# nyasyamorina/font-renderer

Measured on AMD Instinct MI355X. Metric: Mpixel/s AA glyph coverage, higher is better.
Workload: dtype f32

## Files before the change

### bindings/fr_raster.zig

```
const std = @import("std");

const Font = @import("../font/Font.zig");
const Glyph = @import("../font/Glyph.zig");
const Image = @import("Image.zig");
const Point = @import("geometry.zig").Point;

pub const fr_ctx = opaque {};
pub const fr_glyphset = opaque {};
pub const fr_plan = opaque {};
pub const fr_font = opaque {};

pub const Status = enum(c_int) { ok = 0, invalid = -1, hip = -2, nomem = -3, unsupported = -4 };
pub const Mode = enum(i32) { winding_i16 = 0, gray_debug = 1, mask_nonzero = 2, coverage_u8 = 3, sdf_u8 = 4 };
pub const SamplePhase = enum(i32) { corner = 0, center = 1 };
pub const FR_FONT_ALLOW_HINTED: u32 = 1;
pub const FR_FILL_CONSISTENT: u32 = 1;
pub const FR_TEXT_BGRA: u32 = 4;
pub const FR_TEXT_SRGB: u32 = 8;
pub const FR_TEXT_LOAD: u32 = 32;

pub const RasterParams = extern struct {
    mode: i32,
    samples_per_axis: i32,
    sample_phase: i32,
// ... 78 lines not shown
pub extern "c" fn fr_font_close(font: ?*fr_font) void;
pub extern "c" fn fr_font_info(font: *const fr_font, units_per_em: ?*u16, num_glyphs: ?*u16, y0_baseline: ?*c_int) c_int;
pub extern "c" fn fr_font_char_to_glyph(font: *const fr_font, codepoint: u32, glyph_index: *u16) c_int;
pub extern "c" fn fr_font_glyph_advance(font: *const fr_font, glyph_index: u16, advance_width: *i16) c_int;
pub extern "c" fn fr_text_layout(font: *const fr_font, codepoints: [*]const u32, n: u32, font_size: u16, glyph_index_out: [*]u16, pen_x64_out: [*]i32, end_pen_x64: ?*i32) c_int;
pub extern "c" fn fr_font_glyph_measure(font: *fr_font, glyph_index: u16, n_contours: *u32, n_points: *u32, box: *[4]i16) c_int;
pub extern "c" fn fr_font_glyph_fill(font: *fr_font, glyph_index: u16, points_xy: [*]i16, contour_start: [*]u32) c_int;
pub extern "c" fn fr_qoi_bound(width: u32, height: u32) usize;
pub extern "c" fn fr_qoi_encode_rgb(rgb: [*]const u8, width: u32, height: u32, out: [*]u8, cap: usize, n_out: *usize) c_int;
pub extern "c" fn fr_qoi_encode_gray(gray: [*]const u8, width: u32, height: u32, stride: usize, out: [*]u8, cap: usize, n_out: *usize) c_int;
pub extern "c" fn fr_qoi_encode_rgba(rgba: [*]const u8, width: u32, height: u32, stride_px: usize, out: [*]u8, cap: usize, n_out: *usize) c_int;
pub extern "c" fn fr_srgb_decode(in: [*]const u8, n: usize, out: [*]u16) c_int;
pub extern "c" fn fr_srgb_encode(in: [*]const u16, n: usize, out: [*]u8) c_int;
pub extern "c" fn fr_selftest_division(d_lo: u32, d_hi: u32, mismatches: *u64, bad_divisor: ?*u32, bad_x_bits: ?*u32) c_int;
pub extern "c" fn fr_selftest_sqrt(mismatches: *u64, bad_x_bits: ?*u32) c_int;

pub const Error = error{ RasterFailed, OutOfMemory };

var g_ctx: ?*fr_ctx = null;

fn context() Error!*fr_ctx {
    if (g_ctx == null) {
        if (fr_ctx_create(0, null, &g_ctx) != 0) return error.RasterFailed;
    }
    return g_ctx.?;
}

pub fn deinit() void {
    if (g_ctx) |c| fr_ctx_destroy(c);
    g_ctx = null;
// ... 131 lines not shown
```

### font-renderer_amd/_lib.py

```python
from __future__ import annotations

import ctypes as C
import os

FR_WINDING_I16, FR_GRAY_DEBUG, FR_MASK_NONZERO, FR_COVERAGE_U8, FR_SDF_U8 = 0, 1, 2, 3, 4
FR_SAMPLE_CORNER, FR_SAMPLE_CENTER = 0, 1
FR_FILL_CONSISTENT = 1
FR_TEXT_SRGB, FR_TEXT_BGRA = 8, 4
FR_TEXT_LOAD = 32

_HERE = os.path.dirname(os.path.abspath(__file__))


def lib_path() -> str:
    return os.environ.get("FR_RASTER_LIB") or os.path.join(_HERE, "libfr_raster.so")


class FrError(RuntimeError):
    def __init__(self, code: int, msg: str):
        super().__init__(f"fr_raster error {code}: {msg}")
        self.code = code


class Job(C.Structure):
# ... 73 lines not shown
    ("fr_font_open", C.c_int, [_P, C.c_size_t, C.c_uint32, C.POINTER(_P)]),
    ("fr_font_close", None, [_P]),
    ("fr_font_info", C.c_int, [_P, C.POINTER(C.c_uint16), C.POINTER(C.c_uint16), C.POINTER(C.c_int)]),
    ("fr_font_char_to_glyph", C.c_int, [_P, C.c_uint32, C.POINTER(C.c_uint16)]),
    ("fr_font_glyph_advance", C.c_int, [_P, C.c_uint16, C.POINTER(C.c_int16)]),
    ("fr_text_layout", C.c_int, [_P, _P, C.c_uint32, C.c_uint16, _P, _P, C.POINTER(C.c_int32)]),
    ("fr_font_glyph_measure", C.c_int, [_P, C.c_uint16, C.POINTER(C.c_uint32), C.POINTER(C.c_uint32), _P]),
    ("fr_font_glyph_fill", C.c_int, [_P, C.c_uint16, _P, _P]),
    ("fr_qoi_bound", C.c_size_t, [C.c_uint32, C.c_uint32]),
    ("fr_qoi_encode_rgb", C.c_int, [_P, C.c_uint32, C.c_uint32, _P, C.c_size_t, C.POINTER(C.c_size_t)]),
    ("fr_qoi_encode_gray", C.c_int, [_P, C.c_uint32, C.c_uint32, C.c_size_t, _P, C.c_size_t, C.POINTER(C.c_size_t)]),
    ("fr_qoi_encode_rgba", C.c_int, [_P, C.c_uint32, C.c_uint32, C.c_size_t, _P, C.c_size_t, C.POINTER(C.c_size_t)]),
    ("fr_srgb_decode", C.c_int, [_P, C.c_size_t, _P]),
    ("fr_srgb_encode", C.c_int, [_P, C.c_size_t, _P]),
    ("fr_selftest_sqrt", C.c_int, [C.POINTER(C.c_uint64), C.POINTER(C.c_uint32)]),
    ("fr_selftest_division", C.c_int, [C.c_uint32, C.c_uint32, C.POINTER(C.c_uint64), C.POINTER(C.c_uint32), C.POINTER(C.c_uint32)]),
]

_lib = None


def _preload_hip_runtime() -> None:
    if os.environ.get("FR_HIP_RUNTIME", "") == "system":
        return
    import importlib.util
    import sys
    if "torch" in sys.modules:
        return
    try:
        spec = importlib.util.find_spec("torch")
# ... 35 lines not shown
```

### font-renderer_amd/csrc/fr_c4.hpp

```cpp
#pragma once
#include "fr_records.hpp"
#include "fr_wave.hpp"

namespace fr {

#ifndef FR_C4_WAVES
#define FR_C4_WAVES 4
#endif
#ifndef FR_C4_OCC
#define FR_C4_OCC 4
#endif
#ifndef FR_C4_PCAP
#define FR_C4_PCAP 448
#endif
#ifndef FR_C4_OCC_SMALL
#define FR_C4_OCC_SMALL 6
#endif
#ifndef FR_DYN_BANDS
#define FR_DYN_BANDS 1
#endif
#ifndef FR_W1_OCC_SMALL
#define FR_W1_OCC_SMALL 6
#endif
enum { C4_WAVES = FR_C4_WAVES, C4_PCAP = FR_C4_PCAP };
constexpr uint32_t c4_lstride(int cap) { return (uint32_t)cap + 4u; }
constexpr int c4_occ(int cap, int wlog, int rpl) { return rpl >= 16 ? 2 : (rpl >= 8 ? 3 : ((cap <= 16 && rpl == 2) ? FR_C4_OCC_SMALL : FR_C4_OCC)); }
constexpr int w1_occ(int rpl, int wlog) { return rpl >= 16 ? 2 : ((rpl == 2) ? FR_W1_OCC_SMALL : FR_C4_OCC); }
template <uint32_t LSTRIDE>
__device__ __forceinline__ uint4 c4_ld16(const uint16_t *p)
{
    if ((LSTRIDE * 2) % 16 == 0) return *reinterpret_cast<const uint4 *>(p);
    const uint2 a = reinterpret_cast<const uint2 *>(p)[0], b = reinterpret_cast<const uint2 *>(p)[1];
    return make_uint4(a.x, a.y, b.x, b.y);
}
// ... 37 lines not shown
__device__ __forceinline__ Rec40 c4_make_rec40(const Rec &r, uint32_t ra, uint32_t re)
{
    Rec40 m;
    const bool lin = (int32_t)r.flags < 0;
    m.a = lin ? r.c1 : r.a;
    m.b = r.b; m.c1 = lin ? 0.0f : r.c1; m.c2 = r.c2;
    m.ax = r.ax; m.bx = r.bx; m.p0x = r.p0x; m.rden = r.rden;
    m.sgn = r.sqsign ? -1.0f : 1.0f;
    const uint32_t cb = (lin || FILL) ? (r.flags & 2u) : 2u, zb = (lin || FILL) ? cb : 0u;
    m.fr = ra | (re << 12) | (cb << 24) | (zb << 26) | (lin ? 0x80000000u : 0u);
    return m;
}

template <uint32_t RCAP, int N, uint32_t NCOL, int FILL>
__device__ __forceinline__ uint32_t c4_setup_small(const RenderArgs &A, const Job &job, uint32_t seg0, uint32_t nseg, uint32_t x0s,
                                                   int phase, float *s_cxp, Rec40 *s_rec, uint32_t *s_wcnt, uint32_t *s_tmp, const float *cyt = nullptr)
{
    const uint32_t tid = threadIdx.x, lane = tid & 63u, wave = tid >> 6;
    const uint32_t Hs = job.h * (uint32_t)N;
    RowGeom geo;
    geo.max_y = job.max_y; geo.scale = job.scale; geo.rows = Hs; geo.n = N; geo.phase = phase; geo.cyt = cyt;
    const bool have = lane < 2u * nseg;
    Rec r;
    RowGuess g;
    Piece pc;
    g.empty = true; g.ra = 1u; g.re = 0u;
    uint32_t cls = 3u;
    if (have) {
        record_prep<FILL>(A.seg_pts + 6u * (size_t)(seg0 + (lane >> 1)), lane & 1u, geo, r, g, &pc);
        if (!g.empty) {
            const uint32_t row = (wave == 0u) ? g.ra - 1u : (wave == 1u) ? g.ra : (wave == 2u) ? g.re - 1u : g.re;
            if (row < Hs && (wave != 2u || g.re > g.ra)) cls = (uint32_t)row_class<FILL>(r, pc, geo.cy(row));
        }
    }
    s_tmp[tid] = cls;
    const int32_t min_xs = job.min_x + (int32_t)x0s;
    for (uint32_t j = tid; j < NCOL; j += 256u)
        s_cxp[1u + j] = ((float)(min_xs + (int32_t)(j / (uint32_t)N)) + sub_off((int)(j % (uint32_t)N), N, phase)) / job.scale;
    if (tid == 2) s_cxp[0] = -__builtin_inff();
    if (tid == 3) s_cxp[1u + NCOL] = __builtin_inff();
    __syncthreads();
    if (wave == 0u) {
        Rec40 mine;
        mine.fr = 0u;
        bool live = false;
        if (have) {
            uint32_t ra = g.ra, re = g.re;
            if (!g.empty) {
                const uint32_t c0 = s_tmp[lane], c1 = s_tmp[64u + lane], c2 = s_tmp[128u + lane], c3 = s_tmp[192u + lane];
                const bool ok = (c0 >= 2u) && (c1 <= 1u || c1 == 3u) && re >= ra && (c2 >= 1u) && (c3 == 0u || c3 == 3u);
                if (!ok) record_settle<FILL>(r, geo, ra, re, &pc);
            }
            live = ra < re;
// ... 2 lines not shown
        const bool linr = live && (int32_t)mine.fr < 0;
        const unsigned long long lm = __ballot(live && !linr), ll = __ballot(linr), below = (1ull << lane) - 1ull;
        const uint32_t n_quad = (uint32_t)__popcll(lm);
        uint32_t pos = RCAP;
        if ((lm >> lane) & 1ull) pos = (uint32_t)__popcll(lm & below);
        if ((ll >> lane) & 1ull) pos = n_quad + (uint32_t)__popcll(ll & below);
        if (pos < RCAP) s_rec[pos] = mine;
        if (lane == 0u) s_wcnt[0] = min(n_quad + (uint32_t)__popcll(ll), RCAP);
    }
    __syncthreads();
    return s_wcnt[0];
}

template <uint32_t RCAP, int N, uint32_t NCOL, int FILL>
__device__ __forceinline__ uint32_t c4_setup_mid(const RenderArgs &A, const Job &job, uint32_t seg0, uint32_t nseg, uint32_t x0s,
                                                 int phase, float *s_cxp, Rec40 *s_rec, uint32_t *s_wcnt, uint32_t *s_tmp, const float *cyt = nullptr)
{
    const uint32_t tid = threadIdx.x, lane = tid & 63u, wave = tid >> 6;
    const uint32_t c = tid & 127u, h = tid >> 7;
    const uint32_t Hs = job.h * (uint32_t)N;
    RowGeom geo;
    geo.max_y = job.max_y; geo.scale = job.scale; geo.rows = Hs; geo.n = N; geo.phase = phase; geo.cyt = cyt;
    const bool have = c < 2u * nseg;
    Rec r;
    RowGuess g;
    Piece pc;
    g.empty = true; g.ra = 1u; g.re = 0u;
    uint32_t cls0 = 3u, cls1 = 3u;
    if (have) {
        record_prep<FILL>(A.seg_pts + 6u * (size_t)(seg0 + (c >> 1)), c & 1u, geo, r, g, &pc);
        if (!g.empty) {
            const uint32_t end = h ? g.re : g.ra;
            if (end - 1u < Hs && (h == 0u || g.re > g.ra)) cls0 = (uint32_t)row_class<FILL>(r, pc, geo.cy(end - 1u));
            if (end < Hs) cls1 = (uint32_t)row_class<FILL>(r, pc, geo.cy(end));
        }
    }
    s_tmp[tid] = cls0 | (cls1 << 8);
    const int32_t min_xs = job.min_x + (int32_t)x0s;
    for (uint32_t j = tid; j < NCOL; j += 256u)
        s_cxp[1u + j] = ((float)(min_xs + (int32_t)(j / (uint32_t)N)) + sub_off((int)(j % (uint32_t)N), N, phase)) / job.scale;
    if (tid == 2) s_cxp[0] = -__builtin_inff();
    if (tid == 3) s_cxp[1u + NCOL] = __builtin_inff();
    __syncthreads();
    Rec40 mine;
    mine.fr = 0u;
    bool live = false;
    if (h == 0u && have) {
        uint32_t ra = g.ra, re = g.re;
        if (!g.empty) {
            const uint32_t up = s_tmp[c], dn = s_tmp[128u + c];
            const uint32_t c0 = up & 0xffu, c1 = up >> 8, c2 = dn & 0xffu, c3 = dn >> 8;
            const bool ok = (c0 >= 2u) && (c1 <= 1u || c1 == 3u) && re >= ra && (c2 >= 1u) && (c3 == 0u || c3 == 3u);
            if (!ok) record_settle<FILL>(r, geo, ra, re, &pc);
        }
        live = ra < re;
// ... 1 lines not shown
    }
    const bool linr = live && (int32_t)mine.fr < 0;
    const unsigned long long lm = __ballot(live && !linr), ll = __ballot(linr), below = (1ull << lane) - 1ull;
    if (lane == 0u && wave < 2u) { s_wcnt[wave] = (uint32_t)__popcll(lm); s_wcnt[2u + wave] = (uint32_t)__popcll(ll); }
    __syncthreads();
    const uint32_t q0 = s_wcnt[0], q1 = s_wcnt[1], l0 = s_wcnt[2], l1 = s_wcnt[3];
    const uint32_t n_quad = q0 + q1;
    uint32_t pos = RCAP;
    if ((lm >> lane) & 1ull) pos = (wave ? q0 : 0u) + (uint32_t)__popcll(lm & below);
    if ((ll >> lane) & 1ull) pos = n_quad + (wave ? l0 : 0u) + (uint32_t)__popcll(ll & below);
    if (wave < 2u && pos < RCAP) s_rec[pos] = mine;
    __syncthreads();
    return min(n_quad + l0 + l1, RCAP);
}

template <uint32_t NW, uint32_t RCAP, int N, uint32_t NCOL, int FILL = 0>
__device__ __forceinline__ uint32_t c4_setup(const RenderArgs &A, const Job &job, uint32_t seg0, uint32_t nseg, uint32_t x0s,
                                             int phase, float *s_cxp, Rec40 *s_rec, uint32_t *s_wcnt, uint32_t *s_tmp, const float *cyt = nullptr)
{
    if (NW == 4u && 2u * nseg <= 64u)
        return c4_setup_small<RCAP, N, NCOL, FILL>(A, job, seg0, nseg, x0s, phase, s_cxp, s_rec, s_wcnt, s_tmp, cyt);
    if (NW == 4u && 2u * nseg <= 128u)
        return c4_setup_mid<RCAP, N, NCOL, FILL>(A, job, seg0, nseg, x0s, phase, s_cxp, s_rec, s_wcnt, s_tmp, cyt);
    const uint32_t tid = threadIdx.x, lane = tid & 63u, wave = tid >> 6;
    const uint32_t Hs = job.h * (uint32_t)N;
    constexpr uint32_t CPT = (RCAP >= 1024u ? 1536u : (RCAP >= 512u ? 768u : 512u)) / (64u * NW);
    s_wcnt = s_tmp;
    Rec40 mine[CPT];
    unsigned long long lm[CPT], ll[CPT];
#pragma unroll
    for (uint32_t it = 0; it < CPT; ++it) {
        const uint32_t c = tid + it * 64u * NW;
        bool live = false;
        lm[it] = 0ull; ll[it] = 0ull;
        mine[it].fr = 0u;
        if (it > 0 && it * 64u * NW >= 2u * nseg) continue;
        if (c < 2u * nseg) {
            Rec r;
            RowGeom geo;
            geo.max_y = job.max_y; geo.scale = job.scale; geo.rows = Hs; geo.n = N; geo.phase = phase; geo.cyt = cyt;
            build_record_rows<FILL>(A.seg_pts + 6u * (size_t)(seg0 + (c >> 1)), c & 1u, geo, r);
            const uint32_t ra = __builtin_bit_cast(uint32_t, r.lo), re = __builtin_bit_cast(uint32_t, r.hi);
            live = ra < re;
            mine[it] = c4_make_rec40<FILL>(r, ra, re);
        }
        const bool linr = live && (int32_t)mine[it].fr < 0;
        lm[it] = __ballot(live && !linr);
        ll[it] = __ballot(linr);
        if (lane == 0) { s_wcnt[it * NW + wave] = (uint32_t)__popcll(lm[it]); s_wcnt[CPT * NW + it * NW + wave] = (uint32_t)__popcll(ll[it]); }
    }
    const int32_t min_xs = job.min_x + (int32_t)x0s;
    for (uint32_t j = tid; j < NCOL; j += 64u * NW)
        s_cxp[1u + j] = ((float)(min_xs + (int32_t)(j / (uint32_t)N)) + sub_off((int)(j % (uint32_t)N), N, phase)) / job.scale;
    if (tid == 2) s_cxp[0] = -__builtin_inff();
    if (tid == 3) s_cxp[1u + NCOL] = __builtin_inff();
    __syncthreads();
    uint32_t rec_cnt = 0;
    {
        uint32_t base_q[CPT], base_l[CPT], n_quad = 0;
#pragma unroll
        for (uint32_t it = 0; it < CPT; ++it) base_q[it] = base_l[it] = 0;
#pragma unroll
        for (uint32_t q = 0; q < CPT * NW; ++q) {
            if (q >= NW && q / NW * 64u * NW >= 2u * nseg) continue;
            const uint32_t cq = s_wcnt[q], cl = s_wcnt[CPT * NW + q];
#pragma unroll
            for (uint32_t it = 0; it < CPT; ++it) {
                base_q[it] += (q < it * NW + wave) ? cq : 0u;
// ... 21 lines not shown
```

### font-renderer_amd/csrc/fr_cov4_kernel.inc

```
    using L = C4Lds<WLOG, RPL, NS, CAP>;
    constexpr uint32_t LSTRIDE = L::LSTRIDE;
    static_assert(NS == 4 || NS == 2, "samples per axis");
    constexpr uint32_t RCAP = L::RCAP;
    constexpr uint32_t NW = C4_WAVES;
    constexpr uint32_t SW = 16u << WLOG;
    constexpr uint32_t NCOL = SW * (uint32_t)NS;
    constexpr uint32_t NWIN = 1u << WLOG;
    constexpr uint32_t PRB = L::PRB;
    constexpr int LN = (NS == 4) ? 2 : 1;
    constexpr bool SPLIT = RPL >= 8 && CAP == 32;
    extern __shared__ __align__(16) unsigned char smem[];

    const uint32_t tid = threadIdx.x, lane = tid & 63u;
    const uint32_t wave = (uint32_t)__builtin_amdgcn_readfirstlane((int)(tid >> 6));
    uint32_t bid = blockIdx.x, strip = 0, bgrp = 0;
    if (A.strips != 1u) { strip = bid % A.strips; bid /= A.strips; }
    if (A.band_groups != 1u) { bgrp = bid % A.band_groups; bid /= A.band_groups; }
    const uint32_t jidx = bid;
    C4_ABL_LAUNCH_ONLY();
    const Job job = A.jobs[jidx];
    const uint32_t x0s = strip * SW;
    const uint32_t band_first = bgrp * A.bands_per_wg;
    if (band_first * PRB >= job.h || x0s >= job.w) return;
    const uint32_t band_end = min(band_first + A.bands_per_wg, (job.h + PRB - 1u) / PRB);
    const uint32_t wlim = min(SW, job.w - x0s);
    const int phase = A.phase_center;
    const uint32_t seg0 = A.job_seg[2u * (size_t)jidx], nseg = A.job_seg[2u * (size_t)jidx + 1u];
    C4_ABL_JOB_ONLY();
    C4_ABL_SEGLOAD_ONLY();
    float *s_cxp = reinterpret_cast<float *>(smem);
    Rec40 *s_rec = reinterpret_cast<Rec40 *>(smem + L::CX);
    unsigned char *wregion = smem + L::OFF_WAVES + (size_t)wave * L::WAVE;
    uint32_t *s_wcnt = reinterpret_cast<uint32_t *>(smem + L::OFF_WCNT);

    uint32_t *const s_next_band = s_wcnt + 15;
    if (tid == 0u) *s_next_band = band_first + NW;
    const uint32_t rec_cnt = c4_setup<NW, RCAP, NS, NCOL, FILL>(A, job, seg0, nseg, x0s, phase, s_cxp, s_rec, s_wcnt, reinterpret_cast<uint32_t *>(smem + L::OFF_WAVES));
    const int32_t min_xs = job.min_x + (int32_t)x0s;
    const float jscale = job.scale * (float)NS;
    const float joff = (float)min_xs * (float)NS + (phase ? 0.5f : 0.0f) - 1.0f;
    const float ncolf = (float)NCOL;
    const bool few = RPL == 2 || rec_cnt <= 128u;
    const uint32_t per = few ? 2u : (uint32_t)RPL;
    uint32_t rra[RPL], rre[RPL];
#pragma unroll
    for (int i = 0; i < RPL; ++i) {
        const uint32_t k = per * lane + (uint32_t)i;
        const bool have = k < rec_cnt && (!few || i < 2);
        const uint32_t f = s_rec[have ? k : 0u].fr;
        rra[i] = have ? (f & 0xfffu) : 1u;
        rre[i] = have ? ((f >> 12) & 0xfffu) : 0u;
    }
// ... 4 lines not shown
    uint32_t *s_cnt = reinterpret_cast<uint32_t *>(wregion + L::OFF_CNT);
    int16_t *s_roff = reinterpret_cast<int16_t *>(wregion + L::OFF_ROFF);
    unsigned char *s_E = wregion;

    C4_ABL_SETUP_ONLY();
#if FR_DYN_BANDS
    for (uint32_t band = band_first + wave; band < band_end;
         band = (uint32_t)__builtin_amdgcn_readfirstlane((int)(lane == 0u ? atomicAdd(s_next_band, 1u) : 0u))) {
#else
    for (uint32_t band0 = band_first; band0 < band_end; band0 += NW) {
        const uint32_t band = band0 + wave;
        if (band >= band_end) break;
#endif
        const uint32_t y0 = band * PRB;
        const uint32_t row_b0 = band * 64u;
        const float cy = ((float)(job.max_y - (int32_t)(y0 + (lane >> LN))) - sub_off((int)(lane & (uint32_t)(NS - 1)), NS, phase)) / job.scale;
        uint16_t *mylist = s_lists + lane * LSTRIDE;
        auto init_lists = [&]() {
            const uint4 ones = make_uint4(0xfffdfffdu, 0xfffdfffdu, 0xfffdfffdu, 0xfffdfffdu);
#pragma unroll
            for (uint32_t q = 0; q < CAP / 8u; ++q) c4_st16<LSTRIDE>(mylist + 8u * q, ones);
            s_cnt[lane] = 0u;
        };
        init_lists();
        s_cy[lane] = cy;

        uint32_t c[RPL], off0 = 0u, tot;
        {
            uint32_t r0[RPL], csum = 0;
            {
                const uint32_t lo = row_b0, hi = row_b0 + 64u;
// ... 442 lines not shown
```

### font-renderer_amd/csrc/fr_device.hpp

```cpp
#pragma once
#include <hip/hip_runtime.h>
#include <stdint.h>

#pragma clang fp contract(off)

namespace fr {

struct __attribute__((aligned(16))) Rec {
    float lo, hi, a, b, c1, c2, ax, bx, p0x;
    uint32_t flags;
    float rden;
    uint32_t sqsign;
};

__device__ __forceinline__ float div_by_int(float x, float d, float rd)
{
    const float q = x * rd;
    const float r = __builtin_fmaf(-q, d, x);
    return __builtin_fmaf(r, rd, q);
}
__device__ __forceinline__ float sqrt_rn(float x)
{
    const float s = __builtin_amdgcn_sqrtf(x);
    const float sm = __builtin_bit_cast(float, __builtin_bit_cast(int, s) - 1);
    const float sp = __builtin_bit_cast(float, __builtin_bit_cast(int, s) + 1);
    const float rm = __builtin_fmaf(-sm, s, x);
    const float rp = __builtin_fmaf(-sp, s, x);
    float r = (rm <= 0.0f) ? sm : s;
    r = (rp > 0.0f) ? sp : r;
    return r;
}
enum : uint32_t {
    REC_LINEAR = 0x80000000u,
    REC_NEG_ROOT = 2u,
// ... 123 lines not shown
```

### font-renderer_amd/csrc/fr_records.hpp

```cpp
#pragma once
#include "fr_device.hpp"

namespace fr {

__device__ __forceinline__ int classify(const Rec &r, float cy)
{
    if (r.flags & REC_LINEAR) {
        float t = rec_t_lin(r, cy);
        bool up = r.c1 > 0.0f;
        if (t < 0.0f) return up ? 0 : 2;
        if (t >= 1.0f) return up ? 2 : 0;
        return 1;
    }
    float delta = cy * r.a + r.c1 - r.c2;
    if (delta < 0.0f) return (r.a > 0.0f) ? 0 : 2;
    float t = rec_t_quad(r, cy);
    bool neg = (r.flags & REC_NEG_ROOT) != 0;
    if (t < 0.0f) return neg ? 2 : 0;
    if (t >= 1.0f) return neg ? 0 : 2;
    return 1;
}

__device__ __noinline__ uint32_t first_at_least(float ra, float rb, float rc1, float rc2, uint32_t rflags, int T, uint32_t L, uint32_t H)
{
// ... 77 lines not shown
        r.rden = 1.0f / a;
        r.flags = root ? REC_NEG_ROOT : 0u;
    }
    float lo, hi;
    if (!accept_bracket(r, p0y, p2y, lo, hi)) return false;
    r.lo = lo; r.hi = hi;
    return true;
}

struct RowGeom {
    int32_t max_y;
    float scale;
    uint32_t rows;
    int n, phase;
    const float *cyt = nullptr;
    __device__ __forceinline__ float cy(uint32_t r) const
    {
        if (cyt) return cyt[r];
        return ((float)(max_y - (int32_t)(r / (uint32_t)n)) - sub_off((int)(r % (uint32_t)n), n, phase)) / scale;
    }
    __device__ __forceinline__ float row_of(float c) const
    {
        return ((float)max_y - c * scale) * (float)n - (phase ? 0.5f : 0.0f);
    }
};

__device__ __forceinline__ int classify_row(const Rec &r, float cy)
{
    const bool lin = (r.flags & REC_LINEAR) != 0;
    const float delta = cy * r.a + r.c1 - r.c2;
    const float sq = sqrt_rn(delta);
    const float num = lin ? (cy - r.b) : ((r.flags & REC_NEG_ROOT) ? (r.b - sq) : (r.b + sq));
    const float t = div_by_int(num, lin ? r.c1 : r.a, r.rden);
    const bool falls = lin ? !(r.c1 > 0.0f) : ((r.flags & REC_NEG_ROOT) != 0);
// ... 164 lines not shown
```

### font-renderer_amd/csrc/fr_selftest.hip

```cpp
#include "../../include/fr_raster.h"
#include "fr_device.hpp"

namespace fr {

__global__ __launch_bounds__(256) void selftest_div_kernel(uint32_t d_lo, uint32_t n_d,
                                                           unsigned long long *mismatches,
                                                           uint32_t *first_bad)
{
    const uint32_t d_idx = blockIdx.x / 32u, part = blockIdx.x % 32u;
    if (d_idx >= n_d) return;
    const float d = (float)(d_lo + d_idx);
    const float rd = 1.0f / d, rdn = 1.0f / (-d);
    uint32_t bad = 0, bad_x = 0;
    for (uint32_t m = part * 256u + threadIdx.x; m < (1u << 23); m += 32u * 256u) {
        const float x = __uint_as_float(0x3f800000u | m);
        const float xs = __uint_as_float(0x2f800000u | m);
        const float xl = __uint_as_float(0x4f800000u | m);
        const bool ok = (__float_as_uint(div_by_int(x, d, rd)) == __float_as_uint(x / d)) &&
                        (__float_as_uint(div_by_int(x, -d, rdn)) == __float_as_uint(x / -d)) &&
                        (__float_as_uint(div_by_int(-xs, d, rd)) == __float_as_uint(-xs / d)) &&
                        (__float_as_uint(div_by_int(xl, d, rd)) == __float_as_uint(xl / d));
        if (!ok) { ++bad; bad_x = 0x3f800000u | m; }
    }
    if (bad) {
// ... 3 lines not shown
    }
}

__global__ __launch_bounds__(256) void selftest_sqrt_kernel(uint32_t e_lo, unsigned long long *mismatches, uint32_t *first_bad)
{
    const uint32_t e = e_lo + blockIdx.x / 32u, part = blockIdx.x % 32u;
    uint32_t bad = 0, bad_x = 0;
    for (uint32_t m = part * 256u + threadIdx.x; m < (1u << 23); m += 32u * 256u) {
        const uint32_t bits = (e << 23) | m;
        const float x = __uint_as_float(bits);
        if (__float_as_uint(sqrt_rn(x)) != __float_as_uint(__builtin_sqrtf(x))) { ++bad; bad_x = bits; }
    }
    if (bad) {
        atomicAdd(mismatches, (unsigned long long)bad);
        first_bad[0] = bad_x;
    }
}

}

extern "C" int fr_selftest_sqrt(uint64_t *mismatches, uint32_t *bad_x_bits)
{
    if (!mismatches) return FR_E_INVALID;
    unsigned long long *d_m = nullptr;
    uint32_t *d_b = nullptr;
    if (hipMalloc(&d_m, 8) != hipSuccess || hipMalloc(&d_b, 8) != hipSuccess) return FR_E_HIP;
    (void)hipMemset(d_m, 0, 8);
    (void)hipMemset(d_b, 0, 8);
    const uint32_t e_lo = 97u, e_hi = 192u;
    hipLaunchKernelGGL(fr::selftest_sqrt_kernel, dim3((e_hi - e_lo + 1u) * 32u), dim3(256), 0, 0, e_lo, d_m, d_b);
// ... 23 lines not shown
        const uint32_t n = n_d - off < 4096u ? n_d - off : 4096u;
        hipLaunchKernelGGL(fr::selftest_div_kernel, dim3(n * 32u), dim3(256), 0, 0, d_lo + off, n, d_m, d_b);
    }
    unsigned long long m = 0;
    uint32_t b[2] = {0, 0};
    hipError_t e = hipMemcpy(&m, d_m, 8, hipMemcpyDeviceToHost);
    if (e == hipSuccess) e = hipMemcpy(b, d_b, 8, hipMemcpyDeviceToHost);
    (void)hipFree(d_m);
    (void)hipFree(d_b);
    if (e != hipSuccess) return FR_E_HIP;
    *mismatches = m;
    if (bad_divisor) *bad_divisor = b[0];
    if (bad_x_bits) *bad_x_bits = b[1];
    return FR_OK;
}
```

### font-renderer_amd/csrc/fr_win1_kernel.inc

```
    using L = W1Lds<WLOG, RPL>;
    constexpr uint32_t NW = C4_WAVES;
    constexpr uint32_t RCAP = L::RCAP;
    constexpr uint32_t NCOL = L::NCOL;
    constexpr uint32_t NWIN = 1u << WLOG;
    constexpr uint32_t PCAP = L::PCAP;
    constexpr uint32_t ESZ = (MODE == MODE1_WINDING_I16) ? 2u : 1u;
    extern __shared__ __align__(16) unsigned char smem[];

    const uint32_t tid = threadIdx.x, lane = tid & 63u;
    const uint32_t wave = (WLOG == 4 && RPL == 2) ? (tid >> 6) : (uint32_t)__builtin_amdgcn_readfirstlane((int)(tid >> 6));
    uint32_t bid = blockIdx.x, strip = 0, bgrp = 0;
    if (A.strips != 1u) { strip = bid % A.strips; bid /= A.strips; }
    if (A.band_groups != 1u) { bgrp = bid % A.band_groups; bid /= A.band_groups; }
    const uint32_t jidx = bid;
    const Job job = A.jobs[jidx];
    const uint32_t x0s = strip * NCOL;
    const uint32_t band_first = bgrp * A.bands_per_wg;
    if (band_first * W1_ROWS >= job.h || x0s >= job.w) return;
    const uint32_t band_end = min(band_first + A.bands_per_wg, (job.h + W1_ROWS - 1u) / W1_ROWS);
    const uint32_t wlim = min(NCOL, job.w - x0s);
    const int phase = A.phase_center;
    const uint32_t seg0 = A.job_seg[2u * (size_t)jidx], nseg = A.job_seg[2u * (size_t)jidx + 1u];

    float *s_cxp = reinterpret_cast<float *>(smem);
    Rec40 *s_rec = reinterpret_cast<Rec40 *>(smem + L::CX);
    unsigned char *wregion = smem + L::OFF_WAVES + (size_t)wave * L::WAVE;
    uint32_t *s_wcnt = reinterpret_cast<uint32_t *>(smem + L::OFF_WCNT);

    const float soff = phase ? 0.5f : 0.0f;
    const float *cyt = nullptr;
    if (job.h <= 256u) {
        float *t = reinterpret_cast<float *>(smem + L::OFF_CYT);
        if (tid < job.h) t[tid] = ((float)(job.max_y - (int32_t)tid) - soff) / job.scale;
        __syncthreads();
        cyt = t;
    }
    const uint32_t rec_cnt_v = c4_setup<NW, RCAP, 1, NCOL, FILL>(A, job, seg0, nseg, x0s, phase, s_cxp, s_rec, s_wcnt, reinterpret_cast<uint32_t *>(smem + L::OFF_WAVES), cyt);
    const uint32_t rec_cnt = (WLOG == 4 && RPL == 2) ? rec_cnt_v : (uint32_t)__builtin_amdgcn_readfirstlane((int)rec_cnt_v);
    const int32_t min_xs = job.min_x + (int32_t)x0s;
    const float jscale = job.scale;
    const float joff = (float)min_xs + soff - 1.0f;
    const float ncolf = (float)NCOL;
    const bool few = RPL == 2 || rec_cnt <= 128u;
    const uint32_t per = few ? 2u : (uint32_t)RPL;
    uint32_t rra[RPL], rre[RPL];
#pragma unroll
    for (int i = 0; i < RPL; ++i) {
        const uint32_t k = per * lane + (uint32_t)i;
        const bool have = k < rec_cnt && (!few || i < 2);
        const uint32_t f = s_rec[have ? k : 0u].fr;
        rra[i] = have ? (f & 0xfffu) : 1u;
        rre[i] = have ? ((f >> 12) & 0xfffu) : 0u;
    }

    unsigned char *s_E = wregion;
    uint16_t *s_pairs = reinterpret_cast<uint16_t *>(wregion + L::OFF_PAIRS);
    float *s_cy = reinterpret_cast<float *>(wregion + L::OFF_CY);
    uint32_t *s_cnt = reinterpret_cast<uint32_t *>(wregion + L::OFF_CNT);
    int16_t *s_roff = reinterpret_cast<int16_t *>(wregion + L::OFF_ROFF);
    const uint32_t wx = lane & (NWIN - 1u);

    for (uint32_t band0 = band_first; band0 < band_end; band0 += NW) {
        const uint32_t band = band0 + wave;
        if (band >= band_end) break;
        const uint32_t y0 = band * W1_ROWS;
        const float cy = cyt ? cyt[y0 + (lane & 15u)] : ((float)(job.max_y - (int32_t)(y0 + (lane & 15u))) - soff) / job.scale;
        {
            uint4 *z = reinterpret_cast<uint4 *>(s_E);
            const uint4 bias = make_uint4(0x20202020u, 0x20202020u, 0x20202020u, 0x20202020u);
            constexpr uint32_t NZ = L::E / 16u;
#pragma unroll
            for (uint32_t q = 0; q < (NZ + 63u) / 64u; ++q)
                if (NZ % 64u == 0u || lane + 64u * q < NZ) z[lane + 64u * q] = bias;
        }
        if (lane < 16u) { s_cy[lane] = cy; s_cnt[lane] = 0u; }

        uint32_t rr0 = 0;
        while (rr0 < W1_ROWS) {
            uint32_t span = W1_ROWS - rr0;
            uint32_t c[RPL], r0[RPL], csum, incl, tot;
            for (;;) {
// ... 330 lines not shown
```

### include/fr_raster.h

```cpp
#ifndef FR_RASTER_H
#define FR_RASTER_H

#include <stddef.h>
#include <stdint.h>

#ifdef __cplusplus
extern "C" {
#endif

#define FR_ABI_VERSION 1

typedef enum fr_status {
    FR_OK = 0,
    FR_E_INVALID = -1,
    FR_E_HIP = -2,
    FR_E_NOMEM = -3,
    FR_E_UNSUPPORTED = -4
} fr_status;

typedef enum fr_mode {
    FR_WINDING_I16 = 0,
    FR_GRAY_DEBUG = 1,
    FR_MASK_NONZERO = 2,
    FR_COVERAGE_U8 = 3,
// ... 150 lines not shown

int fr_text_layout(const fr_font *font, const uint32_t *codepoints, uint32_t n, uint16_t font_size,
                   uint16_t *glyph_index_out, int32_t *pen_x64_out, int32_t *end_pen_x64);

size_t fr_qoi_bound(uint32_t width, uint32_t height);
int fr_qoi_encode_rgb(const uint8_t *rgb, uint32_t width, uint32_t height, uint8_t *out, size_t cap, size_t *n_out);
int fr_qoi_encode_gray(const uint8_t *gray, uint32_t width, uint32_t height, size_t stride, uint8_t *out, size_t cap, size_t *n_out);
int fr_qoi_encode_rgba(const uint8_t *rgba, uint32_t width, uint32_t height, size_t stride_px, uint8_t *out, size_t cap, size_t *n_out);

int fr_srgb_decode(const uint8_t *in, size_t n, uint16_t *out);
int fr_srgb_encode(const uint16_t *in, size_t n, uint8_t *out);

int fr_selftest_division(uint32_t d_lo, uint32_t d_hi, uint64_t *mismatches,
                         uint32_t *bad_divisor, uint32_t *bad_x_bits);
int fr_selftest_sqrt(uint64_t *mismatches, uint32_t *bad_x_bits);

#ifdef __cplusplus
}
#endif
#endif
```

Baseline: 2.489 million.

## Replace per-row scale divisions with reciprocal refinement and add dense setup path

Replaces the IEEE float divisions by job.scale in row and column coordinate setup with a wave-uniform reciprocal plus two FMA correction steps meant to match division exactly, and adds a selftest that checks this bitwise against true division. It also adds a dense setup path in the cov4 kernel for glyphs with up to 256 segments. That path compacts live records per wave with ballots, then classifies endpoint rows in parallel before settling. The aim is to cut division latency and the serialized setup work per job, at the cost of more code and reliance on the exactness of the refinement.

```diff
diff --git a/bindings/fr_raster.zig b/bindings/fr_raster.zig
--- a/bindings/fr_raster.zig
+++ b/bindings/fr_raster.zig
@@ -116,6 +116,7 @@
 pub extern "c" fn fr_srgb_encode(in: [*]const u16, n: usize, out: [*]u8) c_int;
 pub extern "c" fn fr_selftest_division(d_lo: u32, d_hi: u32, mismatches: *u64, bad_divisor: ?*u32, bad_x_bits: ?*u32) c_int;
 pub extern "c" fn fr_selftest_sqrt(mismatches: *u64, bad_x_bits: ?*u32) c_int;
+pub extern "c" fn fr_selftest_scale_division(mismatches: *u64, bad_scale_bits: ?*u32, bad_x_bits: ?*u32) c_int;
 
 pub const Error = error{ RasterFailed, OutOfMemory };
 
diff --git a/font-renderer_amd/_lib.py b/font-renderer_amd/_lib.py
--- a/font-renderer_amd/_lib.py
+++ b/font-renderer_amd/_lib.py
@@ -111,6 +111,7 @@
     ("fr_srgb_decode", C.c_int, [_P, C.c_size_t, _P]),
     ("fr_srgb_encode", C.c_int, [_P, C.c_size_t, _P]),
     ("fr_selftest_sqrt", C.c_int, [C.POINTER(C.c_uint64), C.POINTER(C.c_uint32)]),
+    ("fr_selftest_scale_division", C.c_int, [C.POINTER(C.c_uint64), C.POINTER(C.c_uint32), C.POINTER(C.c_uint32)]),
     ("fr_selftest_division", C.c_int, [C.c_uint32, C.c_uint32, C.POINTER(C.c_uint64), C.POINTER(C.c_uint32), C.POINTER(C.c_uint32)]),
 ]
 
diff --git a/font-renderer_amd/csrc/fr_c4.hpp b/font-renderer_amd/csrc/fr_c4.hpp
--- a/font-renderer_amd/csrc/fr_c4.hpp
+++ b/font-renderer_amd/csrc/fr_c4.hpp
@@ -18,6 +18,9 @@
 #endif
 #ifndef FR_DYN_BANDS
 #define FR_DYN_BANDS 1
+#endif
+#ifndef FR_C4_DENSE
+#define FR_C4_DENSE 1
 #endif
 #ifndef FR_W1_OCC_SMALL
 #define FR_W1_OCC_SMALL 6
@@ -85,12 +88,12 @@
 
 template <uint32_t RCAP, int N, uint32_t NCOL, int FILL>
 __device__ __forceinline__ uint32_t c4_setup_small(const RenderArgs &A, const Job &job, uint32_t seg0, uint32_t nseg, uint32_t x0s,
-                                                   int phase, float *s_cxp, Rec40 *s_rec, uint32_t *s_wcnt, uint32_t *s_tmp, const float *cyt = nullptr)
+                                                   int phase, float ysc, float *s_cxp, Rec40 *s_rec, uint32_t *s_wcnt, uint32_t *s_tmp, const float *cyt = nullptr)
 {
     const uint32_t tid = threadIdx.x, lane = tid & 63u, wave = tid >> 6;
     const uint32_t Hs = job.h * (uint32_t)N;
     RowGeom geo;
-    geo.max_y = job.max_y; geo.scale = job.scale; geo.rows = Hs; geo.n = N; geo.phase = phase; geo.cyt = cyt;
+    geo.max_y = job.max_y; geo.scale = job.scale; geo.rows = Hs; geo.n = N; geo.phase = phase; geo.cyt = cyt; geo.by_rcp = true; geo.yscale = ysc;
     const bool have = lane < 2u * nseg;
     Rec r;
     RowGuess g;
@@ -107,7 +110,7 @@
     s_tmp[tid] = cls;
     const int32_t min_xs = job.min_x + (int32_t)x0s;
     for (uint32_t j = tid; j < NCOL; j += 256u)
-        s_cxp[1u + j] = ((float)(min_xs + (int32_t)(j / (uint32_t)N)) + sub_off((int)(j % (uint32_t)N), N, phase)) / job.scale;
+        s_cxp[1u + j] = div_by_scale((float)(min_xs + (int32_t)(j / (uint32_t)N)) + sub_off((int)(j % (uint32_t)N), N, phase), job.scale, ysc);
     if (tid == 2) s_cxp[0] = -__builtin_inff();
     if (tid == 3) s_cxp[1u + NCOL] = __builtin_inff();
     __syncthreads();
@@ -140,13 +143,13 @@
 
 template <uint32_t RCAP, int N, uint32_t NCOL, int FILL>
 __device__ __forceinline__ uint32_t c4_setup_mid(const RenderArgs &A, const Job &job, uint32_t seg0, uint32_t nseg, uint32_t x0s,
-                                                 int phase, float *s_cxp, Rec40 *s_rec, uint32_t *s_wcnt, uint32_t *s_tmp, const float *cyt = nullptr)
+                                                 int phase, float ysc, float *s_cxp, Rec40 *s_rec, uint32_t *s_wcnt, uint32_t *s_tmp, const float *cyt = nullptr)
 {
     const uint32_t tid = threadIdx.x, lane = tid & 63u, wave = tid >> 6;
     const uint32_t c = tid & 127u, h = tid >> 7;
     const uint32_t Hs = job.h * (uint32_t)N;
     RowGeom geo;
-    geo.max_y = job.max_y; geo.scale = job.scale; geo.rows = Hs; geo.n = N; geo.phase = phase; geo.cyt = cyt;
+    geo.max_y = job.max_y; geo.scale = job.scale; geo.rows = Hs; geo.n = N; geo.phase = phase; geo.cyt = cyt; geo.by_rcp = true; geo.yscale = ysc;
     const bool have = c < 2u * nseg;
     Rec r;
     RowGuess g;
@@ -164,7 +167,7 @@
     s_tmp[tid] = cls0 | (cls1 << 8);
     const int32_t min_xs = job.min_x + (int32_t)x0s;
     for (uint32_t j = tid; j < NCOL; j += 256u)
-        s_cxp[1u + j] = ((float)(min_xs + (int32_t)(j / (uint32_t)N)) + sub_off((int)(j % (uint32_t)N), N, phase)) / job.scale;
+        s_cxp[1u + j] = div_by_scale((float)(min_xs + (int32_t)(j / (uint32_t)N)) + sub_off((int)(j % (uint32_t)N), N, phase), job.scale, ysc);
     if (tid == 2) s_cxp[0] = -__builtin_inff();
     if (tid == 3) s_cxp[1u + NCOL] = __builtin_inff();
     __syncthreads();
@@ -196,14 +199,119 @@
     return min(n_quad + l0 + l1, RCAP);
 }
 
-template <uint32_t NW, uint32_t RCAP, int N, uint32_t NCOL, int FILL = 0>
+template <uint32_t RCAP, int N, uint32_t NCOL, uint32_t WAVE>
+__device__ __forceinline__ uint32_t c4_setup_dense(const RenderArgs &A, const Job &job, uint32_t seg0, uint32_t nseg, uint32_t x0s,
+                                                   int phase, float ysc, float *s_cxp, Rec40 *s_rec, uint32_t *s_wcnt, unsigned char *s_waves)
+{
+    constexpr uint32_t LIST = 128u * (uint32_t)sizeof(Rec40);
+    static_assert(RCAP == 256u && WAVE >= LIST + RCAP * 4u, "no room for the dense root lists");
+    const uint32_t tid = threadIdx.x, lane = tid & 63u, wave = tid >> 6;
+    const uint32_t Hs = job.h * (uint32_t)N;
+    const unsigned long long below = (1ull << lane) - 1ull;
+    RowGeom geo;
+    geo.max_y = job.max_y; geo.scale = job.scale; geo.rows = Hs; geo.n = N; geo.phase = phase; geo.by_rcp = true; geo.yscale = ysc;
+    uint32_t *s_cls = reinterpret_cast<uint32_t *>(s_waves + LIST);
+    auto rec_of = [](const Rec40 &m) {
+        Rec r;
+        const bool lin = (int32_t)m.fr < 0;
+        r.a = lin ? 0.0f : m.a; r.b = m.b; r.c1 = lin ? m.a : m.c1; r.c2 = m.c2; r.rden = m.rden;
+        r.flags = lin ? (uint32_t)REC_LINEAR : (m.sgn < 0.0f ? (uint32_t)REC_NEG_ROOT : 0u);
+        return r;
+    };
+    {
+        Rec40 e0, e1;
+        bool live0 = false, live1 = false;
+        if (tid < nseg) {
+            const int16_t *p = A.seg_pts + 6u * (size_t)(seg0 + tid);
+            Rec r;
+            RowGuess g;
+            record_prep<0>(p, 0u, geo, r, g);
+            live0 = !g.empty;
+            e0 = c4_make_rec40<0>(r, g.ra, g.re);
+            record_prep<0>(p, 1u, geo, r, g);
+            live1 = !g.empty;
+            e1 = c4_make_rec40<0>(r, g.ra, g.re);
+        }
+        const unsigned long long m0 = __ballot(live0), m1 = __ballot(live1);
+        Rec40 *mylist = reinterpret_cast<Rec40 *>(s_waves + (size_t)wave * WAVE);
+        const uint32_t pos = (uint32_t)__popcll(m0 & below) + (uint32_t)__popcll(m1 & below);
+        if (live0) mylist[pos] = e0;
+        if (live1) mylist[pos + (live0 ? 1u : 0u)] = e1;
+        if (lane == 0u) s_wcnt[wave] = (uint32_t)__popcll(m0) + (uint32_t)__popcll(m1);
+    }
+    const int32_t min_xs = job.min_x + (int32_t)x0s;
+    for (uint32_t j = tid; j < NCOL; j += 256u)
+        s_cxp[1u + j] = div_by_scale((float)(min_xs + (int32_t)(j / (uint32_t)N)) + sub_off((int)(j % (uint32_t)N), N, phase), job.scale, ysc);
+    if (tid == 2) s_cxp[0] = -__builtin_inff();
+    if (tid == 3) s_cxp[1u + NCOL] = __builtin_inff();
+    __syncthreads();
+    const uint32_t cum0 = s_wcnt[0], cum1 = cum0 + s_wcnt[1], cum2 = cum1 + s_wcnt[2];
+    const uint32_t nl = min(cum2 + s_wcnt[3], RCAP);
+    auto entry = [&](uint32_t j) {
+        const uint32_t w = (j >= cum0 ? 1u : 0u) + (j >= cum1 ? 1u : 0u) + (j >= cum2 ? 1u : 0u);
+        const uint32_t first = w == 0u ? 0u : (w == 1u ? cum0 : (w == 2u ? cum1 : cum2));
+        return reinterpret_cast<const Rec40 *>(s_waves + (size_t)w * WAVE) + (j - first);
+    };
+    for (uint32_t i = tid; i < 2u * nl; i += 256u) {
+        const Rec40 *ep = entry(i >> 1);
+        Rec40 m;
+        m.a = ep->a; m.b = ep->b; m.c1 = ep->c1; m.c2 = ep->c2; m.rden = ep->rden; m.sgn = ep->sgn; m.fr = ep->fr;
+        const Rec r = rec_of(m);
+        const Piece pc{};
+        const uint32_t ra = m.fr & 0xfffu, re = (m.fr >> 12) & 0xfffu;
+        const uint32_t end = (i & 1u) ? re : ra;
+        uint32_t cls0 = 3u, cls1 = 3u;
+        if (end - 1u < Hs && ((i & 1u) == 0u || re > ra)) cls0 = (uint32_t)row_class<0>(r, pc, geo.cy(end - 1u));
+        if (end < Hs) cls1 = (uint32_t)row_class<0>(r, pc, geo.cy(end));
+        reinterpret_cast<uint16_t *>(s_cls)[i] = (uint16_t)(cls0 | (cls1 << 8));
+    }
+    __syncthreads();
+    Rec40 mine = {};
+    bool live = false;
+    if (tid < nl) {
+        const Rec40 *ep = entry(tid);
+        mine.a = ep->a; mine.b = ep->b; mine.c1 = ep->c1; mine.c2 = ep->c2; mine.ax = ep->ax; mine.bx = ep->bx; mine.p0x = ep->p0x;
+        mine.rden = ep->rden; mine.sgn = ep->sgn; mine.fr = ep->fr;
+        uint32_t ra = mine.fr & 0xfffu, re = (mine.fr >> 12) & 0xfffu;
+        const uint32_t c4 = s_cls[tid];
+        const uint32_t c0 = c4 & 0xffu, c1 = (c4 >> 8) & 0xffu, c2 = (c4 >> 16) & 0xffu, c3 = c4 >> 24;
+        const bool ok = (c0 >= 2u) && (c1 <= 1u || c1 == 3u) && re >= ra && (c2 >= 1u) && (c3 == 0u || c3 == 3u);
+        if (!ok) record_settle<0>(rec_of(mine), geo, ra, re);
+        live = ra < re;
+        mine.fr = (mine.fr & 0xff000000u) | ra | (re << 12);
+    }
+    const bool linr = live && (int32_t)mine.fr < 0;
+    const unsigned long long lm = __ballot(live && !linr), ll = __ballot(linr);
+    if (lane == 0u) { s_wcnt[4u + wave] = (uint32_t)__popcll(lm); s_wcnt[8u + wave] = (uint32_t)__popcll(ll); }
+    __syncthreads();
+    uint32_t base_q = 0u, base_l = 0u, n_quad = 0u, n_lin = 0u;
+#pragma unroll
+    for (uint32_t w = 0; w < 4u; ++w) {
+        const uint32_t cq = s_wcnt[4u + w], cl = s_wcnt[8u + w];
+        base_q += (w < wave) ? cq : 0u;
+        base_l += (w < wave) ? cl : 0u;
+        n_quad += cq; n_lin += cl;
+    }
+    uint32_t pos = RCAP;
+    if ((lm >> lane) & 1ull) pos = base_q + (uint32_t)__popcll(lm & below);
+    if ((ll >> lane) & 1ull) pos = n_quad + base_l + (uint32_t)__popcll(ll & below);
+    if (pos < RCAP) s_rec[pos] = mine;
+    __syncthreads();
+    return min(n_quad + n_lin, RCAP);
+}
+
+template <uint32_t NW, uint32_t RCAP, int N, uint32_t NCOL, int FILL = 0, uint32_t DENSE_WAVE = 0>
 __device__ __forceinline__ uint32_t c4_setup(const RenderArgs &A, const Job &job, uint32_t seg0, uint32_t nseg, uint32_t x0s,
-                                             int phase, float *s_cxp, Rec40 *s_rec, uint32_t *s_wcnt, uint32_t *s_tmp, const float *cyt = nullptr)
+                                             int phase, float ysc, float *s_cxp, Rec40 *s_rec, uint32_t *s_wcnt, uint32_t *s_tmp, const float *cyt = nullptr)
 {
     if (NW == 4u && 2u * nseg <= 64u)
-        return c4_setup_small<RCAP, N, NCOL, FILL>(A, job, seg0, nseg, x0s, phase, s_cxp, s_rec, s_wcnt, s_tmp, cyt);
+        return c4_setup_small<RCAP, N, NCOL, FILL>(A, job, seg0, nseg, x0s, phase, ysc, s_cxp, s_rec, s_wcnt, s_tmp, cyt);
     if (NW == 4u && 2u * nseg <= 128u)
-        return c4_setup_mid<RCAP, N, NCOL, FILL>(A, job, seg0, nseg, x0s, phase, s_cxp, s_rec, s_wcnt, s_tmp, cyt);
+        return c4_setup_mid<RCAP, N, NCOL, FILL>(A, job, seg0, nseg, x0s, phase, ysc, s_cxp, s_rec, s_wcnt, s_tmp, cyt);
+    if constexpr (DENSE_WAVE != 0u) {
+        if (nseg <= 256u)
+            return c4_setup_dense<RCAP, N, NCOL, DENSE_WAVE>(A, job, seg0, nseg, x0s, phase, ysc, s_cxp, s_rec, s_wcnt, reinterpret_cast<unsigned char *>(s_tmp));
+    }
     const uint32_t tid = threadIdx.x, lane = tid & 63u, wave = tid >> 6;
     const uint32_t Hs = job.h * (uint32_t)N;
     constexpr uint32_t CPT = (RCAP >= 1024u ? 1536u : (RCAP >= 512u ? 768u : 512u)) / (64u * NW);
@@ -220,7 +328,7 @@
         if (c < 2u * nseg) {
             Rec r;
             RowGeom geo;
-            geo.max_y = job.max_y; geo.scale = job.scale; geo.rows = Hs; geo.n = N; geo.phase = phase; geo.cyt = cyt;
+            geo.max_y = job.max_y; geo.scale = job.scale; geo.rows = Hs; geo.n = N; geo.phase = phase; geo.cyt = cyt; geo.by_rcp = true; geo.yscale = ysc;
             build_record_rows<FILL>(A.seg_pts + 6u * (size_t)(seg0 + (c >> 1)), c & 1u, geo, r);
             const uint32_t ra = __builtin_bit_cast(uint32_t, r.lo), re = __builtin_bit_cast(uint32_t, r.hi);
             live = ra < re;
@@ -233,7 +341,7 @@
     }
     const int32_t min_xs = job.min_x + (int32_t)x0s;
     for (uint32_t j = tid; j < NCOL; j += 64u * NW)
-        s_cxp[1u + j] = ((float)(min_xs + (int32_t)(j / (uint32_t)N)) + sub_off((int)(j % (uint32_t)N), N, phase)) / job.scale;
+        s_cxp[1u + j] = div_by_scale((float)(min_xs + (int32_t)(j / (uint32_t)N)) + sub_off((int)(j % (uint32_t)N), N, phase), job.scale, ysc);
     if (tid == 2) s_cxp[0] = -__builtin_inff();
     if (tid == 3) s_cxp[1u + NCOL] = __builtin_inff();
     __syncthreads();
diff --git a/font-renderer_amd/csrc/fr_cov4_kernel.inc b/font-renderer_amd/csrc/fr_cov4_kernel.inc
--- a/font-renderer_amd/csrc/fr_cov4_kernel.inc
+++ b/font-renderer_amd/csrc/fr_cov4_kernel.inc
@@ -35,7 +35,9 @@
 
     uint32_t *const s_next_band = s_wcnt + 15;
     if (tid == 0u) *s_next_band = band_first + NW;
-    const uint32_t rec_cnt = c4_setup<NW, RCAP, NS, NCOL, FILL>(A, job, seg0, nseg, x0s, phase, s_cxp, s_rec, s_wcnt, reinterpret_cast<uint32_t *>(smem + L::OFF_WAVES));
+    const float ysc = scale_rcp_uniform(job.scale);
+    constexpr uint32_t DENSE_WAVE = (FR_C4_DENSE && FILL == 0 && RPL == 4 && NW == 4u && L::WAVE >= 128u * (uint32_t)sizeof(Rec40) + RCAP * 4u) ? L::WAVE : 0u;
+    const uint32_t rec_cnt = c4_setup<NW, RCAP, NS, NCOL, FILL, DENSE_WAVE>(A, job, seg0, nseg, x0s, phase, ysc, s_cxp, s_rec, s_wcnt, reinterpret_cast<uint32_t *>(smem + L::OFF_WAVES));
     const int32_t min_xs = job.min_x + (int32_t)x0s;
     const float jscale = job.scale * (float)NS;
     const float joff = (float)min_xs * (float)NS + (phase ? 0.5f : 0.0f) - 1.0f;
@@ -70,7 +72,7 @@
 #endif
         const uint32_t y0 = band * PRB;
         const uint32_t row_b0 = band * 64u;
-        const float cy = ((float)(job.max_y - (int32_t)(y0 + (lane >> LN))) - sub_off((int)(lane & (uint32_t)(NS - 1)), NS, phase)) / job.scale;
+        const float cy = div_by_scale((float)(job.max_y - (int32_t)(y0 + (lane >> LN))) - sub_off((int)(lane & (uint32_t)(NS - 1)), NS, phase), job.scale, ysc);
         uint16_t *mylist = s_lists + lane * LSTRIDE;
         auto init_lists = [&]() {
             const uint4 ones = make_uint4(0xfffdfffdu, 0xfffdfffdu, 0xfffdfffdu, 0xfffdfffdu);
diff --git a/font-renderer_amd/csrc/fr_device.hpp b/font-renderer_amd/csrc/fr_device.hpp
--- a/font-renderer_amd/csrc/fr_device.hpp
+++ b/font-renderer_amd/csrc/fr_device.hpp
@@ -18,6 +18,22 @@
     const float q = x * rd;
     const float r = __builtin_fmaf(-q, d, x);
     return __builtin_fmaf(r, rd, q);
+}
+__device__ __forceinline__ float scale_rcp(float d)
+{
+    const float y0 = __builtin_amdgcn_rcpf(d);
+    return __builtin_fmaf(__builtin_fmaf(-d, y0, 1.0f), y0, y0);
+}
+__device__ __forceinline__ float scale_rcp_uniform(float d)
+{
+    return __builtin_bit_cast(float, __builtin_amdgcn_readfirstlane(__builtin_bit_cast(int, scale_rcp(d))));
+}
+__device__ __forceinline__ float div_by_scale(float x, float d, float y)
+{
+    float q = x * y;
+    q = __builtin_fmaf(__builtin_fmaf(-d, q, x), y, q);
+    q = __builtin_fmaf(__builtin_fmaf(-d, q, x), y, q);
+    return q;
 }
 __device__ __forceinline__ float sqrt_rn(float x)
 {
diff --git a/font-renderer_amd/csrc/fr_records.hpp b/font-renderer_amd/csrc/fr_records.hpp
--- a/font-renderer_amd/csrc/fr_records.hpp
+++ b/font-renderer_amd/csrc/fr_records.hpp
@@ -115,10 +115,13 @@
     uint32_t rows;
     int n, phase;
     const float *cyt = nullptr;
+    bool by_rcp = false;
+    float yscale = 0.0f;
     __device__ __forceinline__ float cy(uint32_t r) const
     {
         if (cyt) return cyt[r];
-        return ((float)(max_y - (int32_t)(r / (uint32_t)n)) - sub_off((int)(r % (uint32_t)n), n, phase)) / scale;
+        const float num = (float)(max_y - (int32_t)(r / (uint32_t)n)) - sub_off((int)(r % (uint32_t)n), n, phase);
+        return by_rcp ? div_by_scale(num, scale, yscale) : num / scale;
     }
     __device__ __forceinline__ float row_of(float c) const
     {
diff --git a/font-renderer_amd/csrc/fr_selftest.hip b/font-renderer_amd/csrc/fr_selftest.hip
--- a/font-renderer_amd/csrc/fr_selftest.hip
+++ b/font-renderer_amd/csrc/fr_selftest.hip
@@ -41,6 +41,25 @@
     if (bad) {
         atomicAdd(mismatches, (unsigned long long)bad);
         first_bad[0] = bad_x;
+    }
+}
+
+__global__ __launch_bounds__(256) void selftest_scale_div_kernel(uint32_t e, uint32_t m_lo, uint32_t n_m, const float *__restrict__ xs, uint32_t n_x,
+                                                                  unsigned long long *mismatches, uint32_t *first_bad)
+{
+    const uint32_t i = blockIdx.x * 256u + threadIdx.x;
+    if (i >= n_m) return;
+    const uint32_t dbits = (e << 23) | (m_lo + i);
+    const float d = __uint_as_float(dbits);
+    const float y = scale_rcp(d);
+    uint32_t bad = 0, bad_x = 0;
+    for (uint32_t k = 0; k < n_x; ++k) {
+        const float x = xs[k];
+        if (__float_as_uint(div_by_scale(x, d, y)) != __float_as_uint(x / d)) { if (!bad) bad_x = __float_as_uint(x); ++bad; }
+    }
+    if (bad) {
+        atomicAdd(mismatches, (unsigned long long)bad);
+        if (atomicMin(&first_bad[0], dbits) > dbits) first_bad[1] = bad_x;
     }
 }
 
@@ -94,3 +113,63 @@
     if (bad_x_bits) *bad_x_bits = b[1];
     return FR_OK;
 }
+
+static void scale_div_numerators(float *xs, uint32_t n)
+{
+    uint32_t at = 0;
+    auto put = [&](float v) { if (at < n) xs[at++] = v; };
+    put(0.0f);
+    for (int k = 1; k < 8; ++k) { put((float)k / 8.0f); put(-(float)k / 8.0f); }
+    const int32_t ext[] = {1, 2, 3, 2047, 2048, 32767, 32768, 34816, 65535, 65536, (1 << 22) - 1, 1 << 22};
+    for (int32_t i : ext)
+        for (int k = 0; k < 8; k += (i < 4 ? 1 : 7)) {
+            put((float)i + (float)k / 8.0f); put((float)i - (float)k / 8.0f);
+            put((float)-i + (float)k / 8.0f); put((float)-i - (float)k / 8.0f);
+        }
+    uint64_t st = 0x9e3779b97f4a7c15ull;
+    auto next = [&]() { st += 0x9e3779b97f4a7c15ull; uint64_t z = st; z = (z ^ (z >> 30)) * 0xbf58476d1ce4e5b9ull; z = (z ^ (z >> 27)) * 0x94d049bb133111ebull; return z ^ (z >> 31); };
+    while (at < n) {
+        const uint64_t r = next();
+        const uint32_t bits = 1u + (uint32_t)(r % 22u);
+        int32_t i = (int32_t)((r >> 8) & ((1u << bits) - 1u));
+        if (r & (1ull << 40)) i = -i;
+        const float off = (float)((r >> 44) & 7u) / 8.0f;
+        put((r & (1ull << 48)) ? (float)i + off : (float)i - off);
+    }
+}
+
+extern "C" int fr_selftest_scale_division(uint64_t *mismatches, uint32_t *bad_scale_bits, uint32_t *bad_x_bits)
+{
+    if (!mismatches) return FR_E_INVALID;
+    enum { NX = 2048 };
+    static float xs[NX];
+    scale_div_numerators(xs, NX);
+    unsigned long long *d_m = nullptr;
+    uint32_t *d_b = nullptr;
+    float *d_x = nullptr;
+    if (hipMalloc(&d_m, 8) != hipSuccess || hipMalloc(&d_b, 8) != hipSuccess || hipMalloc(&d_x, sizeof xs) != hipSuccess) return FR_E_HIP;
+    const uint32_t init[2] = {0xffffffffu, 0u};
+    hipError_t e = hipMemset(d_m, 0, 8);
+    if (e == hipSuccess) e = hipMemcpy(d_b, init, 8, hipMemcpyHostToDevice);
+    if (e == hipSuccess) e = hipMemcpy(d_x, xs, sizeof xs, hipMemcpyHostToDevice);
+    if (e == hipSuccess) {
+        const uint32_t NM = 1u << 23;
+        hipLaunchKernelGGL(fr::selftest_scale_div_kernel, dim3(NM / 256u), dim3(256), 0, 0, 127u, 0u, NM, d_x, (uint32_t)NX, d_m, d_b);
+        hipLaunchKernelGGL(fr::selftest_scale_div_kernel, dim3(NM / 256u), dim3(256), 0, 0, 107u, 0u, NM, d_x, (uint32_t)NX, d_m, d_b);
+        hipLaunchKernelGGL(fr::selftest_scale_div_kernel, dim3(NM / 256u), dim3(256), 0, 0, 146u, 0u, NM, d_x, (uint32_t)NX, d_m, d_b);
+        hipLaunchKernelGGL(fr::selftest_scale_div_kernel, dim3(1), dim3(256), 0, 0, 147u, 0u, 1u, d_x, (uint32_t)NX, d_m, d_b);
+        e = hipGetLastError();
+    }
+    unsigned long long m = 0;
+    uint32_t b[2] = {0, 0};
+    if (e == hipSuccess) e = hipMemcpy(&m, d_m, 8, hipMemcpyDeviceToHost);
+    if (e == hipSuccess) e = hipMemcpy(b, d_b, 8, hipMemcpyDeviceToHost);
+    (void)hipFree(d_m);
+    (void)hipFree(d_b);
+    (void)hipFree(d_x);
+    if (e != hipSuccess) return FR_E_HIP;
+    *mismatches = m;
+    if (bad_scale_bits) *bad_scale_bits = m ? b[0] : 0u;
+    if (bad_x_bits) *bad_x_bits = m ? b[1] : 0u;
+    return FR_OK;
+}
diff --git a/font-renderer_amd/csrc/fr_win1_kernel.inc b/font-renderer_amd/csrc/fr_win1_kernel.inc
--- a/font-renderer_amd/csrc/fr_win1_kernel.inc
+++ b/font-renderer_amd/csrc/fr_win1_kernel.inc
@@ -28,14 +28,15 @@
     uint32_t *s_wcnt = reinterpret_cast<uint32_t *>(smem + L::OFF_WCNT);
 
     const float soff = phase ? 0.5f : 0.0f;
+    const float ysc = scale_rcp_uniform(job.scale);
     const float *cyt = nullptr;
     if (job.h <= 256u) {
         float *t = reinterpret_cast<float *>(smem + L::OFF_CYT);
-        if (tid < job.h) t[tid] = ((float)(job.max_y - (int32_t)tid) - soff) / job.scale;
+        if (tid < job.h) t[tid] = div_by_scale((float)(job.max_y - (int32_t)tid) - soff, job.scale, ysc);
         __syncthreads();
         cyt = t;
     }
-    const uint32_t rec_cnt_v = c4_setup<NW, RCAP, 1, NCOL, FILL>(A, job, seg0, nseg, x0s, phase, s_cxp, s_rec, s_wcnt, reinterpret_cast<uint32_t *>(smem + L::OFF_WAVES), cyt);
+    const uint32_t rec_cnt_v = c4_setup<NW, RCAP, 1, NCOL, FILL>(A, job, seg0, nseg, x0s, phase, ysc, s_cxp, s_rec, s_wcnt, reinterpret_cast<uint32_t *>(smem + L::OFF_WAVES), cyt);
     const uint32_t rec_cnt = (WLOG == 4 && RPL == 2) ? rec_cnt_v : (uint32_t)__builtin_amdgcn_readfirstlane((int)rec_cnt_v);
     const int32_t min_xs = job.min_x + (int32_t)x0s;
     const float jscale = job.scale;
@@ -64,7 +65,7 @@
         const uint32_t band = band0 + wave;
         if (band >= band_end) break;
         const uint32_t y0 = band * W1_ROWS;
-        const float cy = cyt ? cyt[y0 + (lane & 15u)] : ((float)(job.max_y - (int32_t)(y0 + (lane & 15u))) - soff) / job.scale;
+        const float cy = cyt ? cyt[y0 + (lane & 15u)] : div_by_scale((float)(job.max_y - (int32_t)(y0 + (lane & 15u))) - soff, job.scale, ysc);
         {
             uint4 *z = reinterpret_cast<uint4 *>(s_E);
             const uint4 bias = make_uint4(0x20202020u, 0x20202020u, 0x20202020u, 0x20202020u);
diff --git a/include/fr_raster.h b/include/fr_raster.h
--- a/include/fr_raster.h
+++ b/include/fr_raster.h
@@ -188,6 +188,7 @@
 int fr_selftest_division(uint32_t d_lo, uint32_t d_hi, uint64_t *mismatches,
                          uint32_t *bad_divisor, uint32_t *bad_x_bits);
 int fr_selftest_sqrt(uint64_t *mismatches, uint32_t *bad_x_bits);
+int fr_selftest_scale_division(uint64_t *mismatches, uint32_t *bad_scale_bits, uint32_t *bad_x_bits);
 
 #ifdef __cplusplus
 }
```

Result: slower. 2.368 million (-4.9%).
